# LPMP/BDD

Measured on AMD Instinct MI355X. Metric: parallel-MMA iterations/sec, 10.5M BDD nodes, 1 GPU (+ achieved HBM GB/s in roofline), higher is better.
Workload: dtype f32

## Files before the change

bdd_amd/capi.py:

```python
from __future__ import annotations

import ctypes as C
import os
import subprocess

_HERE = os.path.dirname(os.path.abspath(__file__))
LIB_PATH = os.path.abspath(os.environ["BDDMMA_LIB"]) if os.environ.get("BDDMMA_LIB") else os.path.join(_HERE, "csrc", "libbdd_mma_hip.so")

OK = 0
ERR_INVALID_ARGUMENT, ERR_INVALID_BDD, ERR_DEVICE, ERR_STATE, ERR_UNSUPPORTED, ERR_IO = -1, -2, -3, -4, -5, -6
F32, F64 = 0, 1
K_FORWARD_MM, K_BACKWARD_MM, K_FINISH_DELTA, K_OTHER, K_COUNT = 0, 1, 2, 3, 4


class Options(C.Structure):
    _fields_ = [("pack_width", C.c_uint32), ("wide_pack_width", C.c_uint32), ("deterministic", C.c_uint32),
                ("vars_per_bin", C.c_uint32), ("stage_cap", C.c_uint32), ("waves_per_block", C.c_uint32),
                ("keep_bdd_order", C.c_uint32), ("resident_sweeps", C.c_uint32), ("exchange_by_variable", C.c_uint32),
                ("variant_flags", C.c_uint32), ("pack_fill", C.c_uint32), ("pack_stagger", C.c_uint32)]


class LbfgsParams(C.Structure):
    _fields_ = [("history_size", C.c_int32), ("init_step_size", C.c_double), ("req_rel_lb_increase", C.c_double),
                ("step_size_decrease_factor", C.c_double), ("step_size_increase_factor", C.c_double)]
# ... 5 lines not shown
                ("last_kind", C.c_int32), ("last_trials", C.c_int32)]


class RunResult(C.Structure):
    _fields_ = [("iterations", C.c_uint64), ("lb_initial", C.c_double), ("lb_final", C.c_double),
                ("seconds", C.c_double), ("stop_reason", C.c_int32)]


class Profile(C.Structure):
    _fields_ = [("launches", C.c_uint64 * K_COUNT), ("total_ms", C.c_double * K_COUNT)]


_V, _U64, _I, _D = C.c_void_p, C.c_uint64, C.c_int, C.c_double
SIGNATURES = {
    "bddmma_create": (_I, [C.POINTER(_V), _I, _I, _V, _V, _U64, _V, _U64, C.POINTER(Options)]),
    "bddmma_destroy": (None, [_V]),
    "bddmma_device_count": (_I, []),
    "bddmma_device_chip": (_I, [_I, C.POINTER(C.c_uint32), C.POINTER(C.c_uint32), C.POINTER(C.c_uint64)]),
    "bddmma_set_layout_threads": (_I, [_I]),
    "bddmma_set_thread_layout_threads": (_I, [_I]),
    "bddmma_last_error": (C.c_char_p, [_V]),
    "bddmma_nr_variables": (_U64, [_V]),
    "bddmma_nr_bdds": (_U64, [_V]),
    "bddmma_nr_layers": (_U64, [_V]),
    "bddmma_nr_bdd_nodes": (_U64, [_V]),
    "bddmma_nr_hops": (_U64, [_V]),
    "bddmma_nr_packs": (_U64, [_V]),
    "bddmma_solve_sweep_kind": (_I, [_V]),
    "bddmma_fused_small": (_I, [_V]),
    "bddmma_fused_small_learned": (_I, [_V]),
    "bddmma_fused_small_history": (_I, [_V]),
    "bddmma_nontemporal_loads": (_I, [_V]),
    "bddmma_potentials_on_chip": (_I, [_V]),
    "bddmma_precision": (_I, [_V]),
    "bddmma_device": (_I, [_V]),
    "bddmma_num_bdds_per_var": (_I, [_V, _V]),
    "bddmma_layer_variables": (_I, [_V, _V]),
    "bddmma_layer_bdds": (_I, [_V, _V]),
    "bddmma_nodes_per_hop": (_I, [_V, _V]),
    "bddmma_layers_per_hop": (_I, [_V, _V]),
    "bddmma_update_costs": (_I, [_V, _V, _U64, _V, _U64, _I, _I]),
    "bddmma_set_cost": (_I, [_V, _D, _U64]),
    "bddmma_get_solver_costs": (_I, [_V, _V, _V, _V, _I]),
    "bddmma_set_solver_costs": (_I, [_V, _V, _V, _V, _I]),
    "bddmma_primal_objective_vec": (_I, [_V, _V, _I]),
    "bddmma_forward_run": (_I, [_V]),
    "bddmma_backward_run": (_I, [_V]),
    "bddmma_lower_bound": (_I, [_V, C.POINTER(_D)]),
    "bddmma_lower_bound_per_bdd": (_I, [_V, _V, _I]),
    "bddmma_iteration": (_I, [_V, _D]),
    "bddmma_iterations": (_I, [_V, _D, _U64]),
    "bddmma_learned_iterations": (_I, [_V, _V, _I, _U64, _D, _D, _V, _V, _V, _U64, _D, _I, C.POINTER(_U64)]),
    "bddmma_learned_iterations_omega_vec": (_I, [_V, _V, _I, _U64, _V, _I, _D, _V, _V, _V, _U64, _D, _I, C.POINTER(_U64)]),
    "bddmma_isotropic_dist_weights": (_I, [_V, _V, _I]),
    "bddmma_forward_mm": (_I, [_V, _D, _V, _I]),
    "bddmma_backward_mm": (_I, [_V, _D, _V, _I]),
    "bddmma_normalize_delta": (_I, [_V, _V, _I]),
    "bddmma_distribute_delta": (_I, [_V]),
    "bddmma_get_delta": (_I, [_V, _V, _I]),
    "bddmma_set_delta": (_I, [_V, _V, _I]),
    "bddmma_min_marginals": (_I, [_V, _I, _V, _V, _V, _I]),
    "bddmma_min_marginal_diff": (_I, [_V, _V, _I]),
    "bddmma_sum_marginals": (_I, [_V, _I, _I, _V, _V, _V, _I]),
    "bddmma_smooth_solution": (_I, [_V, _V, _I]),
    "bddmma_grad_min_marginal_diff": (_I, [_V, _V, _V, _V, _I]),
    "bddmma_grad_lower_bound_per_bdd": (_I, [_V, _V, _V, _V, _I, _I]),
# ... 119 lines not shown
```

bdd_amd/csrc/capi.cpp:

```cpp
#include <chrono>
#include <cmath>
#include <cstdio>
#include <cstdlib>
#include <cstring>
#include <limits>
#include <new>
#include <string>
#include <vector>

#include "../../include/bdd_mma.h"
#include "layout.hpp"
#include "solver.hpp"

using namespace bddmma;

struct bddmma_lbfgs;
extern "C" int bddmma_lbfgs_iteration(bddmma_lbfgs* l);
extern "C" int bddmma_lbfgs_update_costs(bddmma_lbfgs* l, const void* lo, uint64_t n_lo, const void* hi, uint64_t n_hi, int elem_precision,
                                         int on_device);

namespace {
thread_local std::string g_err;

template <typename F>
// ... 101 lines not shown
{
    if (n < 0) return BDDMMA_ERR_INVALID_ARGUMENT;
    set_layout_threads((unsigned)n);
    return BDDMMA_OK;
}
int bddmma_set_thread_layout_threads(int n)
{
    if (n < 0) return BDDMMA_ERR_INVALID_ARGUMENT;
    set_thread_layout_threads((unsigned)n);
    return BDDMMA_OK;
}

void bddmma_destroy(bddmma_solver* s)
{
    if (!s) return;
    delete s->impl;
    delete s;
}

const char* bddmma_last_error(const bddmma_solver* s) { return (s && s->impl) ? s->impl->err.c_str() : g_err.c_str(); }

uint64_t bddmma_nr_variables(const bddmma_solver* s) { return s && s->impl ? s->impl->n_vars : 0; }
uint64_t bddmma_nr_bdds(const bddmma_solver* s) { return s && s->impl ? s->impl->n_bdds : 0; }
uint64_t bddmma_nr_layers(const bddmma_solver* s) { return s && s->impl ? s->impl->n_layers : 0; }
uint64_t bddmma_nr_bdd_nodes(const bddmma_solver* s) { return s && s->impl ? s->impl->n_input_nodes : 0; }
uint64_t bddmma_nr_hops(const bddmma_solver* s) { return s && s->impl ? s->impl->n_hops : 0; }
uint64_t bddmma_nr_packs(const bddmma_solver* s) { return s && s->impl ? s->impl->n_packs_narrow + s->impl->n_packs_wide : 0; }
int bddmma_solve_sweep_kind(const bddmma_solver* s) { return s && s->impl ? s->impl->solve_sweep_kind : -1; }
int bddmma_fused_small(const bddmma_solver* s) { return s && s->impl ? (s->impl->fused_small ? 1 : 0) : -1; }
int bddmma_fused_small_learned(const bddmma_solver* s) { return s && s->impl ? (s->impl->fused_small_learned ? 1 : 0) : -1; }
int bddmma_fused_small_history(const bddmma_solver* s) { return s && s->impl ? (s->impl->fused_small_history ? 1 : 0) : -1; }
int bddmma_nontemporal_loads(const bddmma_solver* s) { return s && s->impl ? (s->impl->nt_loads ? 1 : 0) : -1; }
int bddmma_potentials_on_chip(const bddmma_solver* s) { return s && s->impl ? (s->impl->pot_on_chip ? 1 : 0) : -1; }
int bddmma_precision(const bddmma_solver* s) { return s && s->impl ? s->impl->precision : -1; }
int bddmma_device(const bddmma_solver* s) { return s && s->impl ? s->impl->device : -1; }
uint64_t bddmma_device_bytes(const bddmma_solver* s) { return s && s->impl ? s->impl->dev_bytes : 0; }
uint64_t bddmma_device_allocated_bytes(const bddmma_solver* s) { return s && s->impl ? s->impl->dev_alloc_bytes : 0; }

int bddmma_num_bdds_per_var(const bddmma_solver* s, int32_t* out)
{
    return guarded(s, [&](SolverBase* b) { return copy_host(b->h_nbdds, out); });
}
int bddmma_layer_variables(const bddmma_solver* s, int32_t* out)
{
    return guarded(s, [&](SolverBase* b) { return copy_host(b->h_layer_var, out); });
}
int bddmma_layer_bdds(const bddmma_solver* s, int32_t* out)
{
    return guarded(s, [&](SolverBase* b) { return copy_host(b->h_layer_bdd, out); });
}
int bddmma_nodes_per_hop(const bddmma_solver* s, uint64_t* out)
{
    return guarded(s, [&](SolverBase* b) { return copy_host(b->nodes_per_hop, out); });
}
int bddmma_layers_per_hop(const bddmma_solver* s, uint64_t* out)
{
    return guarded(s, [&](SolverBase* b) { return copy_host(b->layers_per_hop, out); });
}

int bddmma_update_costs(bddmma_solver* s, const void* lo, uint64_t n_lo, const void* hi, uint64_t n_hi,
                        int elem_precision, int on_device)
{
    return guarded(s, [&](SolverBase* b) {
        if (elem_precision != BDDMMA_F32 && elem_precision != BDDMMA_F64) {
            b->err = "elem_precision must be BDDMMA_F32 or BDDMMA_F64";
            return BDDMMA_ERR_INVALID_ARGUMENT;
// ... 670 lines not shown
```

bdd_amd/csrc/kernels/narrow4.hpp:

```cpp
#pragma once

namespace bddmma {

template <typename REAL, int WPB, int HC, bool REBUILD_T, bool STORE_F>
__device__ __forceinline__ void fwd_narrow4_body(const DevPtrs<REAL>& d, const PackDev& pk, const uint32_t* __restrict__ lrec,
                                                 const uint32_t* __restrict__ lrec_off, uint32_t lrec_words, REAL omega, uint32_t block_id)
{
    static_assert(HC + 1 <= (int)HOP_WIN, "one window of hop offsets has to hold the pack");
    constexpr int W = N3_W;
    constexpr uint32_t S = sizeof(REAL);
    constexpr uint32_t BUF = (W + 128) * S;
    using P2 = typename Pair<REAL>::type;
    extern __shared__ __attribute__((aligned(16))) unsigned char dyn_lds[];
    P2* sD = reinterpret_cast<P2*>(dyn_lds);
    __shared__ __attribute__((aligned(16))) unsigned char sF_[WPB][2][BUF];
    __shared__ __attribute__((aligned(16))) unsigned char sT_[WPB][2][BUF];
    __shared__ uint32_t sOffN_[WPB][HOP_WIN], sOffL_[WPB][HOP_WIN], sOffR_[WPB][HOP_WIN];
    const uint32_t tid = threadIdx.x;
    const int wave = __builtin_amdgcn_readfirstlane((int)(tid >> 6));
    const int lane = tid & 63;
    unsigned char* sFw = &sF_[wave][0][0];
    unsigned char* sTw = &sT_[wave][0][0];
    const uint32_t n_quads = (pk.n_packs + WPB - 1) / WPB;
    const uint32_t quad = block_to_pack(block_id, n_quads, pk.xcd_chunk);
    BDDMMA_EXIT_IF(quad >= n_quads, d)
    const uint32_t p = quad * WPB + wave;
    const bool has_pack = p < pk.n_packs;
    const uint32_t* const hp = pk.hdr_pack + 8 * (size_t)(has_pack ? p : 0);
    const uint32_t q0 = !has_pack ? 0 : hp[4];
    const uint32_t hops = !has_pack ? 0 : (hp[5] & 0xFFFFu);
    const uint32_t q1 = q0 + hops;
    const uint32_t rbase = has_pack ? lrec_off[p] : 0;
    const uint32_t c0_h = pk.hdr_quad[4 * (size_t)quad], cnt = pk.hdr_quad[4 * (size_t)quad + 1];
    BDDMMA_STAMP(p, 0);
    const REAL INF = inf_v<REAL>();
    const uint32_t slot_first = !has_pack ? 0 : hp[0], l0 = !has_pack ? 0 : hp[2];
    NarrowRs<REAL> rs(d);
    rs.rebase_layers(d, l0);
    uint32_t ent[STAGE_ITERS], esl[STAGE_ITERS];
    stage_load_tables<REAL, WPB, BDDMMA_LD_TAB_AUX>(ent, esl, rs, c0_h, cnt, tid);
    REAL* const Tp = d.T + slot_first;
    REAL* const Fp = d.F + slot_first;
    const REAL* const lohi_p = d.lohi + 2 * (size_t)l0;
    const rsrc_t rr = make_rsrc(lrec, lrec_words);
    HopWindow hw{sOffN_[wave], sOffL_[wave], sOffR_[wave], q0, q1, slot_first, l0};
    uint32_t o[HC + 4];
    uint32_t lb[HC + 1];
    P2 L[HC];
    P2 T[HC + 2];
#pragma unroll
    for (int i = 0; i < HC + 4; ++i) o[i] = 0;
#pragma unroll
    for (int i = 0; i < HC + 1; ++i) lb[i] = 0;
#pragma unroll
    for (int i = 0; i < HC + 2; ++i) T[i] = P2{REAL(0), REAL(0)};
    auto ldrec = [&](uint32_t h) { return __builtin_amdgcn_raw_buffer_load_b128(rr, (uint32_t)lane * 16u, (rbase + h * 64u) * 16u, 0); };
    const uint32_t sink = (W + 2 * (uint32_t)lane) * S;
    u4v rA = u4v{0u, 0u, 0u, 0u}, rB = rA;
    const uint32_t db = (uint32_t)wave * pk.stage_cap * (uint32_t)sizeof(P2);
    if (has_pack) {
        hw.fill(pk, q0, lane);
#pragma unroll
        for (int i = 0; i < HC + 4; ++i) o[i] = hw.node_off(q0 + i);
#pragma unroll
        for (int i = 0; i < HC + 1; ++i) lb[i] = hw.layer_off(q0 + i);
#pragma unroll
        for (int h = 0; h < HC; ++h)
            hop_load(L[h], rs.lohi, (uint32_t)h < hops ? (uint32_t)lane * (uint32_t)sizeof(P2) : OOB, lb[h] * (uint32_t)sizeof(P2));
        if constexpr (!REBUILD_T) {
#pragma unroll
            for (int h = 1; h < HC; ++h) pot_pair_load<REAL, false>(T[h], hop_rsrc(Tp, o[h], o[h + 1] - o[h]), 2u * (uint32_t)lane * S, o[h] * S);
        }
#pragma unroll
        for (int r = 0; r < 2; ++r) {
            const uint32_t j = lane + 64 * r;
            lds_st<REAL>(sFw, j * S, (j < o[1] - o[0]) ? REAL(0) : INF);
        }
#pragma unroll
        for (int b = 0; b < 2; ++b) {
            lds_st<REAL>(sTw, b * BUF + sink, REAL(0));
            lds_st<REAL>(sTw, b * BUF + sink + S, INF);
        }
        wave_sync();
        if constexpr (REBUILD_T) {
            rA = ldrec(hops - 1);
            rB = ldrec(hops >= 2 ? hops - 2 : 0);
#pragma unroll
            for (int h = HC - 1; h >= 1; --h) {
                if ((uint32_t)h < hops) {
                    const u4v ra = rA;
                    rA = rB;
                    rB = ldrec(h >= 2 ? h - 2 : 0);
                    const uint32_t tc = ((h + 1) & 1) * BUF, tn = (h & 1) * BUF;
                    const P2 c = L[h];
                    const uint32_t flags = ra[2] >> 16;
                    const REAL tla = lds_ld<REAL>(sTw, tc + (ra[0] & 0xFFFFu)), tha = lds_ld<REAL>(sTw, tc + (ra[0] >> 16));
                    const REAL tlb = lds_ld<REAL>(sTw, tc + (ra[1] & 0xFFFFu)), thb = lds_ld<REAL>(sTw, tc + (ra[1] >> 16));
                    const REAL ta = rmin(c.y + tha, c.x + tla);
                    const REAL tb = rmin(c.y + thb, c.x + tlb);
                    if (flags & LREC_REAL) lds_st<REAL>(sTw, tn + (ra[2] & 0xFFFFu), ta);
                    if (flags & LREC_TWO) lds_st<REAL>(sTw, tn + (ra[2] & 0xFFFFu) + S, tb);
                    wave_sync();
                    T[h] = lds_ld<P2>(sTw, tn + 2u * (uint32_t)lane * S);
                }
            }
        } else {
            if (2u * (uint32_t)lane < o[2] - o[1]) lds_st<P2>(sTw, BUF + 2u * (uint32_t)lane * S, T[1]);
        }
        rA = ldrec(0);
        rB = ldrec(1);
    }
    stage_load_pairs<REAL, WPB>(sD, ent, esl, rs, cnt, tid);
    if (WPB > 1) __syncthreads(); else wave_sync();
    BDDMMA_STAMP(p, 1);
#pragma unroll
    for (int h = 0; h < HC; ++h) {
        if ((uint32_t)h < hops) {
            const u4v ra = rA;
            rA = rB;
            rB = ldrec(h + 2);
            const uint32_t fc = (h & 1) * BUF, fn = ((h + 1) & 1) * BUF;
            const uint32_t stg = db + (lb[h] + (uint32_t)lane) * (uint32_t)sizeof(P2);
            const P2 c = L[h];
            const uint32_t flags = ra[2] >> 16;
            REAL fa, fb;
            lds_ld2(fa, fb, sFw, fc + (ra[2] & 0xFFFFu));
            const REAL tla = lds_ld<REAL>(sTw, fn + (ra[0] & 0xFFFFu)), tha = lds_ld<REAL>(sTw, fn + (ra[0] >> 16));
            const REAL tlb = lds_ld<REAL>(sTw, fn + (ra[1] & 0xFFFFu)), thb = lds_ld<REAL>(sTw, fn + (ra[1] >> 16));
            const P2 dd = lds_ld<P2>(dyn_lds, stg);
            if (!(REBUILD_T && h == 0))
                if (2u * (uint32_t)lane < o[h + 3] - o[h + 2]) lds_st<P2>(sTw, fc + 2u * (uint32_t)lane * S, T[h + 2]);
            lds_st<P2>(sFw, fn + 2u * (uint32_t)lane * S, P2{INF, INF});
            wave_sync();
            fa = (flags & LREC_REAL) ? fa : INF;
            fb = (flags & LREC_TWO) ? fb : INF;
            const REAL m0 = rmin((fa + c.x) + tla, (fb + c.x) + tlb);
            const REAL m1 = rmin((fa + c.y) + tha, (fb + c.y) + thb);
            const REAL mm = mm_diff1(m0, m1, omega);
            P2 nc;
            nc.x = (c.x + min0(mm)) + dd.x;
            nc.y = (c.y + min0_neg(mm)) + dd.y;
            const rsrc_t rl = hop_rsrc(reinterpret_cast<const P2*>(lohi_p), lb[h], lb[h + 1] - lb[h]);
            hop_store(nc, rl, (uint32_t)lane * (uint32_t)sizeof(P2), lb[h] * (uint32_t)sizeof(P2));
            if (flags & LREC_REAL) lds_st<REAL>(dyn_lds, stg, mm);
            lds_min(reinterpret_cast<REAL*>(sFw + fn + (ra[0] & 0xFFFFu)), fa + nc.x);
            lds_min(reinterpret_cast<REAL*>(sFw + fn + (ra[0] >> 16)), fa + nc.y);
            lds_min(reinterpret_cast<REAL*>(sFw + fn + (ra[1] & 0xFFFFu)), fb + nc.x);
            lds_min(reinterpret_cast<REAL*>(sFw + fn + (ra[1] >> 16)), fb + nc.y);
            if constexpr (STORE_F) {
                const rsrc_t rf = hop_rsrc(Fp, o[h], o[h + 1] - o[h]);
                pot_store_layer<REAL>(fa, fb, (flags & LREC_TWO) != 0, rf, ra[3] & 0xFFFFu, o[h] * S, pk.nt_potentials);
            }
            wave_sync();
        }
    }
    BDDMMA_STAMP(p, 3);
    if (WPB > 1) __syncthreads(); else wave_sync();
    BDDMMA_STAMP(p, 2);
    stage_flush<REAL, WPB>(sD, ent, esl, rs, cnt, tid);
    BDDMMA_STAMP(p, 4);
}

template <typename REAL, int WPB, int HC, bool REBUILD_T, bool STORE_F>
// ... 185 lines not shown
```

bdd_amd/csrc/solver.hpp:

```cpp
#pragma once
#include <hip/hip_runtime.h>

#include <cstdint>
#include <limits>
#include <memory>
#include <string>
#include <utility>
#include <vector>

#include "../../include/bdd_mma.h"
#include "layout.hpp"

namespace bddmma {

struct SolverBase {
    int precision = BDDMMA_F32, device = -1;
    hipStream_t stream = nullptr;
    std::string err;
    uint64_t n_vars = 0, n_bdds = 0, n_layers = 0, n_hops = 0, n_input_nodes = 0, n_slots = 0;
    int solve_sweep_kind = 0;
    uint32_t pack_width = 0, wide_pack_width = 0, wide_slot_base = 0;
    uint64_t dev_bytes = 0;
    uint64_t dev_alloc_bytes = 0;
    bool fwd_valid = false, bwd_valid = false;
// ... 15 lines not shown
    bool prof_active = false;
    std::vector<std::pair<hipEvent_t, hipEvent_t>> ev_pool;
    std::vector<int> ev_class;
    size_t ev_used = 0;
    hipEvent_t ev_t0 = nullptr, ev_t1 = nullptr;
    hipEvent_t ev_order = nullptr;

    virtual ~SolverBase() {}
    virtual int forward_run() = 0;
    virtual int backward_run() = 0;
    virtual int lower_bound(double* lb) = 0;
    virtual int lower_bound_enqueue(int slot) = 0;
    virtual int lower_bound_fetch(int slot, double* lb) = 0;
    virtual int lower_bound_per_bdd(void* out, int on_device) = 0;
    virtual int iteration(double omega) = 0;
    virtual int iterations(double omega, uint64_t n)
    {
        for (uint64_t i = 0; i < n; ++i)
            if (int rc = iteration(omega)) return rc;
        return BDDMMA_OK;
    }
    virtual int learned_iterations(const void* dist_weights, int weights_on_device, uint64_t num_itr, double omega, double improvement_slope,
                                   void* sol_avg, void* lb_first_diff_avg, void* lb_second_diff_avg, uint64_t compute_history_for_itr,
                                   double history_avg_beta, int outputs_on_device, uint64_t* itr_done, const void* omega_vec,
                                   int omega_vec_on_device) = 0;
    virtual int isotropic_dist_weights(void* out, int on_device) = 0;
    double initial_lb_change = std::numeric_limits<double>::infinity();
    std::shared_ptr<int> lbfgs_attached = std::make_shared<int>(0);
    bool fused_small = false;
    bool fused_small_learned = false;
    bool fused_small_history = false;
    bool nt_loads = false;
    bool pot_on_chip = false;
    virtual int run_plain(uint64_t max_iter, double tolerance, double slope, double time_limit, int verbose, bddmma_run_result* res) = 0;
    virtual int forward_mm(double omega, void* delta, int on_device) = 0;
    virtual int backward_mm(double omega, void* delta, int on_device) = 0;
    virtual int normalize_delta(void* delta, int on_device) = 0;
    virtual int distribute_delta() = 0;
    virtual int get_delta(void* out, int on_device) = 0;
    virtual int set_delta(const void* in, int on_device) = 0;
    virtual int update_costs(const void* lo, uint64_t n_lo, const void* hi, uint64_t n_hi, int elem_precision, int on_device) = 0;
    virtual int set_cost(double c, uint64_t var) = 0;
    virtual int get_solver_costs(void* lo, void* hi, void* mm, int on_device) = 0;
    virtual int set_solver_costs(const void* lo, const void* hi, const void* mm, int on_device) = 0;
    virtual int primal_objective_vec(void* out, int on_device) = 0;
    virtual int min_marginals(int sorted, int32_t* var, void* mm0, void* mm1, int on_device) = 0;
    virtual int min_marginal_diff(void* out, int on_device) = 0;
    virtual int sum_marginals(int sorted, int log_probs, int32_t* var, void* sm0, void* sm1, int on_device) = 0;
    virtual int smooth_solution(void* out, int on_device) = 0;
    virtual int grad_min_marginal_diff(const void* grad_mm, void* grad_lo, void* grad_hi, int on_device) = 0;
    virtual int grad_lower_bound_per_bdd(const void* grad_lb, void* grad_lo, void* grad_hi, int smooth, int on_device) = 0;
    virtual int grad_distribute_delta(const void* grad_lo, const void* grad_hi, void* grad_deferred_mm, int on_device) = 0;
    virtual int grad_cost_perturbation(const void* grad_lo, const void* grad_hi, void* grad_lo_pert, void* grad_hi_pert, int on_device) = 0;
    virtual int grad_learned_iterations(const void* dist_weights, int weights_on_device, double omega, const void* omega_vec, int omega_vec_on_device,
                                        void* grad_lo, void* grad_hi, void* grad_mm, void* grad_dist_weights_out, void* grad_omega_out, uint64_t after,
                                        uint64_t n, uint64_t num_caches, int on_device) = 0;
    virtual int bdds_solution(int sorted, char* sol, int on_device) = 0;
    virtual int net_solver_costs(void* out, int on_device) = 0;
    virtual int make_dual_feasible(void* g, int on_device) = 0;
    virtual int gradient_step(const void* g, double step, int on_device) = 0;
    virtual int projection_means(const void* g_dev) = 0;
    virtual int gradient_step_projected(const void* g_dev, double step) = 0;
    virtual bool projection_fuses_lincomb() const = 0;
    virtual int projection_means_lincomb(const LinComb& lc, const void* tag) = 0;
    virtual void* stream_handle() = 0;
    struct LbfgsViews {
// ... 54 lines not shown
```

bdd_amd/csrc/solver_impl.hpp:

```cpp
#pragma once
#include <hip/hip_runtime.h>
#include <atomic>
#include <chrono>
#include <cmath>
#include <cstdio>
#include <cstdlib>
#include <cstring>
#include <limits>
#include <memory>
#include <string>
#include <thread>
#include <type_traits>
#include <vector>
#include "../../include/bdd_mma.h"
#include "kernels.hpp"
#include "layout.hpp"
#include "solver.hpp"

namespace bddmma {

static inline void cpu_relax()
{
#if defined(__x86_64__) || defined(__i386__)
    __asm__ __volatile__("pause");
// ... 442 lines not shown
                srec_words = (uint32_t)SR.rec.size();
                use_narrow2 = true;
                narrow_gen = narrow_seg;
                for (uint16_t r : L.narrow.hop_root) narrow_gen = narrow_gen || r != NO_ROOT;
            }
        }
        if (nb_.n_packs && !use_res && !wb_.n_packs && !hb_.n_packs && !narrow_seg && pack_width == 128 && (L.ex.waves_per_block == 4 || L.ex.waves_per_block == 8) &&
            !(opts && (opts->variant_flags & 0x41000u))) {
            LayerRecords LR;
            build_layer_records(L, sizeof(REAL), LR);
            const uint32_t n3_static = L.ex.waves_per_block * (4 * (128 + 128) * (uint32_t)sizeof(REAL) + 3 * 64 * 4);
            const bool forced = opts && (opts->variant_flags & 0x2000u);
            const bool shared = forced || (LR.rec.size() * sizeof(uint32_t) <= (uint64_t)L.narrow_slots * sizeof(REAL) / 2 && n_slots <= 16'000'000ull);
            if (LR.ok && shared && stage_lds + n3_static <= lds_cu - 1024) {
                if ((rc = upload(&d_lrec, LR.rec))) return rc;
                if ((rc = upload(&d_lrec_off, LR.rec_off))) return rc;
                lrec_words = (uint32_t)LR.rec.size();
                use_narrow3 = true;
                n3_nt = sizeof(REAL) == 8 && nt_potentials != 0;
            }
        }
        if (nb_.n_packs && !use_res && !use_narrow3 && !wb_.n_packs && !hb_.n_packs && !narrow_seg && !narrow_gen && pack_width == 128 &&
            (L.ex.waves_per_block == 4 || L.ex.waves_per_block == 8) && (beyond_cache || (opts && (opts->variant_flags & 0x100000u))))
#ifndef BDDMMA_EXP_NO_N12_NT
            n12_nt = !use_narrow2 || sizeof(REAL) == 8;
#else
            n12_nt = false;
#endif
        nt_loads = n3_nt || n12_nt;
        if constexpr (sizeof(REAL) == 4) {
            if (use_narrow3 && res_hdr_ok && !n3_nt && !(opts && (opts->variant_flags & 0x200000u))) {
                uint32_t max_hops = 0;
                for (uint32_t p = 0; p < nb_.n_packs; ++p) max_hops = std::max(max_hops, L.res.pack_hdr[8 * (size_t)p + 5] & 0xFFFFu);
                onchip_hc = max_hops <= 10 ? 10 : max_hops <= 16 ? 16 : 0;
                const uint32_t part = opts ? (opts->variant_flags >> 22) & 3u : 0u;
                if (onchip_hc == 16) onchip_mode = 3;
                if (part == 1 || part == 2) {
                    if (onchip_hc == 10 && wpb == 4) onchip_mode = part;
                    else onchip_hc = 0;
                }
                pot_on_chip = onchip_hc != 0;
            }
        }
        if (wb_.n_packs) {
            wide_threads = std::min<uint32_t>(1024, std::max<uint32_t>(64, ((wide_pack_width + 1) / 2 + 63) / 64 * 64));
            wide_npt = (wide_pack_width + wide_threads - 1) / wide_threads;
            wide_npt = wide_npt <= 1 ? 1 : (wide_npt <= 2 ? 2 : 4);
            wide_lds = (uint32_t)wide2_lds_bytes(sizeof(REAL), wide_pack_width, true);
            if (wide_lds > lds_cu || wide_pack_width > 4096) {
                err = "wide_pack_width " + std::to_string(wide_pack_width) + " needs " + std::to_string(wide_lds) + " B of LDS (> 160 KiB)";
                return BDDMMA_ERR_UNSUPPORTED;
            }
        }
        if (wb_.n_packs && nb_.n_packs && !use_res && !(opts && (opts->variant_flags & 1u))) {
            const uint32_t threads = 64 * wpb;
            const uint32_t npt = (wide_pack_width + threads - 1) / threads;
            const uint32_t narrow_dyn = stage_lds + seg_bytes(wpb);
            if (npt <= 4 && wide_lds <= narrow_dyn + 16 * 1024 && std::max(narrow_dyn, wide_lds) + narrow_static <= 64 * 1024) {
                mixed = true;
                mixed_npt = npt <= 1 ? 1 : (npt <= 2 ? 2 : 4);
                mixed_lds = std::max(narrow_dyn, wide_lds);
            }
        }
        if (use_res2 && res_hdr_ok && nb_.n_packs <= SMALL_MAX_PACKS && !wb_.n_packs && !hb_.n_packs && !deterministic && !entry_by_var && !big &&
            L.var_ptr.size() == n_vars + 1 && L.ex.vpos.size() == n_layers && !(opts && (opts->variant_flags & 0x80000u))) {
            const uint32_t np = nb_.n_packs;
            std::vector<uint32_t> lds_off(n_layers);
            uint32_t max_hops = 0;
            bool ok = true;
            for (uint32_t k = 0; k < (uint32_t)n_layers && ok; ++k) {
                const uint32_t l = L.var_layers[k];
                uint32_t p = 0;
                while (p < np && !(l >= L.res.pack_hdr[8 * (size_t)p + 2] && l < L.res.pack_hdr[8 * (size_t)p + 2] + L.res.pack_hdr[8 * (size_t)p + 3])) ++p;
                if (p == np || l - L.res.pack_hdr[8 * (size_t)p + 2] >= res2_nl) { ok = false; break; }
// ... 152 lines not shown
                    if (use_res && use_res2) s.res2 = bwd ? &k_bwd_res2<REAL, W, OV> : &k_fwd_res2<REAL, W, OV>;
                    else if (use_res) s.res = bwd ? &k_bwd_res<REAL, R, W, OV> : &k_fwd_res<REAL, R, W, OV>;
                    else if (use_narrow3 && w48) {
                        s.rec = bwd ? &k_bwd_narrow3<REAL, W48, false, OV> : &k_fwd_narrow3<REAL, W48, false, OV>;
                        if constexpr (sizeof(REAL) == 8)
                            if (n3_nt) s.rec = bwd ? &k_bwd_narrow3<REAL, W48, true, OV> : &k_fwd_narrow3<REAL, W48, true, OV>;
                        s.rec_tab = d_lrec; s.rec_off = d_lrec_off; s.rec_words = lrec_words;
                    } else if (use_narrow2) {
                        if (n12_nt && R == 2 && w48) s.rec = bwd ? &k_bwd_narrow2<REAL, 2, W48, false, sizeof(REAL) == 8, OV> : &k_fwd_narrow2<REAL, 2, W48, false, sizeof(REAL) == 8, OV>;
                        else if (narrow_gen) s.rec = bwd ? &k_bwd_narrow2<REAL, R, W, true, false, OV> : &k_fwd_narrow2<REAL, R, W, true, false, OV>;
                        else s.rec = bwd ? &k_bwd_narrow2<REAL, R, W, false, false, OV> : &k_fwd_narrow2<REAL, R, W, false, false, OV>;
                        s.rec_tab = d_srec; s.rec_off = d_srec_off; s.rec_words = srec_words;
                    } else if (n12_nt && R == 2 && w48) s.narrow = bwd ? &k_bwd_narrow<REAL, 2, MODE, W48, false, true, OV> : &k_fwd_narrow<REAL, 2, MODE, W48, false, true, OV>;
                    else if (!narrow_seg) s.narrow = bwd ? &k_bwd_narrow<REAL, R, MODE, W, false, false, OV> : &k_fwd_narrow<REAL, R, MODE, W, false, false, OV>;
                    else s.narrow = bwd ? &k_bwd_narrow<REAL, R, MODE, W, true, false, OV> : &k_fwd_narrow<REAL, R, MODE, W, true, false, OV>;
                });
            });
            if (mixed)
                s.mixed = {pick<64, 128, 256>(pack_width, [&](auto PW) {
                               return pick<1, 2, 4, 8>(wpb, [&](auto W) {
                                   return pick<1, 2, 4>(mixed_npt, [&](auto N) -> MixedFn {
                                       constexpr int R = PW.value / 64;
                                       return bwd ? &k_bwd_mixed<REAL, R, W.value, N.value, OV> : &k_fwd_mixed<REAL, R, W.value, N.value, OV>;
                                   });
                               });
                           }),
                           mixed_lds};
        }
        return s;
    }
    RecFn onchip_fn(bool bwd, bool rebuild, bool store) const
    {
        if (onchip_hc == 16) return pick<4, 8>(wpb, [&](auto W) -> RecFn { return &k_bwd_narrow4<REAL, W.value, 16, true, true>; });
        if (rebuild && !store)
            return pick<4, 8>(wpb, [&](auto W) -> RecFn {
                return bwd ? &k_bwd_narrow4<REAL, W.value, 10, true, false> : &k_fwd_narrow4<REAL, W.value, 10, true, false>;
            });
        if (rebuild) return bwd ? &k_bwd_narrow4<REAL, 4, 10, true, true> : &k_fwd_narrow4<REAL, 4, 10, true, true>;
        return bwd ? &k_bwd_narrow4<REAL, 4, 10, false, false> : &k_fwd_narrow4<REAL, 4, 10, false, false>;
    }
    void resolve_kernels()
    {
        for (int bwd = 0; bwd < 2; ++bwd) {
            kern.sweep[bwd][FWD_PLAIN] = resolve_sweep<FWD_PLAIN, false>(bwd);
            kern.sweep[bwd][FWD_SOLVE] = resolve_sweep<FWD_SOLVE, false>(bwd);
            kern.sweep[bwd][FWD_SOLUTION] = resolve_sweep<FWD_SOLUTION, false>(bwd);
        }
        if (onchip_hc) {
            for (int bwd = 0; bwd < 2; ++bwd) {
                Sweep s = kern.sweep[bwd][FWD_SOLVE];
                if (onchip_mode == 3 && !bwd) { kern.onchip[0] = s; continue; }
                const bool rebuild = onchip_mode == 0 || (onchip_mode == 1) == !bwd;
                const bool store = onchip_mode != 0 && rebuild;
                if constexpr (sizeof(REAL) == 4) s.rec = onchip_fn(bwd, rebuild, onchip_mode == 3 || store);
                s.reads_pot = !rebuild;
                s.stores_pot = onchip_mode == 3 || store;
                kern.onchip[bwd] = s;
            }
        }
        kern.ex_threads = exch_small ? EXS_THREADS : exch_medium ? EXM_THREADS : EX_THREADS;
        pick<EXS_THREADS, EXM_THREADS, EX_THREADS>(kern.ex_threads, [&](auto T_) {
            constexpr int T = T_.value, U = T == EXS_THREADS ? EXS_UNROLL : T == EXM_THREADS ? EXM_UNROLL : EX_UNROLL,
                          N = T == EXS_THREADS ? EXS_NPT : T == EXM_THREADS ? EXM_NPT : EX_NPT;
            kern.ex[0] = {&k_exchange_reduce<REAL, BDDMMA_EX_ACC, EX_ITER, T, U, N, false>, exch_lds};
            kern.ex[1] = {&k_exchange_reduce<REAL, BDDMMA_EX_ACC, EX_ITER, T, U, N, true>, exch_lds};
            kern.ex_w = {&k_exchange_reduce<REAL, BDDMMA_EX_ACC, EX_ITER, T, U, N, false, true>, exch_lds};
// ... 1161 lines not shown
    {
        const uint64_t n4 = BDDMMA_TRIAD_BYTES / 16;
        stream_v4 *a = nullptr, *b = nullptr, *c = nullptr;
        HIPCHK(hipMalloc(&a, BDDMMA_TRIAD_BYTES));
        HIPCHK(hipMalloc(&b, BDDMMA_TRIAD_BYTES));
        HIPCHK(hipMalloc(&c, BDDMMA_TRIAD_BYTES));
        HIPCHK(hipMemsetAsync(b, 0, BDDMMA_TRIAD_BYTES, stream));
        HIPCHK(hipMemsetAsync(c, 0, BDDMMA_TRIAD_BYTES, stream));
        const unsigned grid = (unsigned)((n4 + 255) / 256);
        auto once = [&]() {
            if (copy) k_stream<true><<<grid, 256, 0, stream>>>(a, b, c, 3.0f, n4);
            else k_stream<false><<<grid, 256, 0, stream>>>(a, b, c, 3.0f, n4);
        };
        once();
        HIPCHK(hipEventRecord(ev_t0, stream));
        for (uint64_t i = 0; i < reps; ++i) once();
        HIPCHK(hipEventRecord(ev_t1, stream));
        HIPCHK(hipEventSynchronize(ev_t1));
        float f = 0.f;
        HIPCHK(hipEventElapsedTime(&f, ev_t0, ev_t1));
        *ms = f;
        HIPCHK(hipFree(a));
        HIPCHK(hipFree(b));
        HIPCHK(hipFree(c));
        return BDDMMA_OK;
    }

    int time_kernel(int kind, uint64_t reps, double* ms) override
    {
        HIPCHK(hipSetDevice(device));
        if (kind >= 13 && kind <= 17) return gi_time_kernel(kind, reps, ms);
        int rc = BDDMMA_OK;
        auto once = [&]() -> int {
            switch (kind) {
                case 0: return launch_fwd(FWD_PLAIN, nullptr, REAL(0), BDDMMA_K_OTHER);
                case 1: return launch_bwd(BWD_PLAIN, nullptr, REAL(0), BDDMMA_K_OTHER);
                case 2: return launch_fwd(FWD_SOLVE, d_delta_lay, REAL(0.5), BDDMMA_K_OTHER);
                case 3: return launch_bwd(BWD_SOLVE, d_delta_lay, REAL(0.5), BDDMMA_K_OTHER);
                case 4: return exchange();
                case 5: launch_bcast(d_delta_c, d_delta_lay_c); return BDDMMA_OK;
                case 8: return sm_launch_fwd();
                case 9: return sm_launch_bwd();
                case 10: return gr_launch_down();
                case 11: return gr_launch_up();
                case 12: { const int r = gr_launch_down(); return r ? r : gr_launch_up(); }
                default: err = "unknown kernel kind"; return BDDMMA_ERR_INVALID_ARGUMENT;
            }
        };
        if (kind == 6 || kind == 7) return time_stream(kind == 7, reps, ms);
        if ((kind == 8 || kind == 9) && (rc = sm_prepare())) return rc;
        if (kind == 9 && (rc = sm_launch_fwd())) return rc;
        if (kind >= 10 && kind <= 12) {
            if ((rc = gr_prepare()) || (rc = forward_run()) || (rc = backward_run())) return rc;
            HIPCHK(hipMemsetAsync(d_gr_in0, 0, n_layers * sizeof(REAL), stream));
            if (kind == 11 && (rc = gr_launch_down())) return rc;
        }
        if ((rc = once())) return rc;
        HIPCHK(hipEventRecord(ev_t0, stream));
        for (uint64_t i = 0; i < reps; ++i)
            if ((rc = once())) return rc;
        HIPCHK(hipEventRecord(ev_t1, stream));
        HIPCHK(hipEventSynchronize(ev_t1));
        float f = 0.f;
        HIPCHK(hipEventElapsedTime(&f, ev_t0, ev_t1));
        *ms = f;
        costs_changed();
        x_layer_valid = false;
#ifdef BDDMMA_STAMPS
        if (const char* path = std::getenv("BDDMMA_STAMPS_FILE")) {
            const size_t slots = 0x100000u + 65536u * 16u;
            unsigned long long* d_st = nullptr;
            HIPCHK(hipMalloc((void**)&d_st, slots * 8 * sizeof(unsigned long long)));
            HIPCHK(hipMemset(d_st, 0, slots * 8 * sizeof(unsigned long long)));
            HIPCHK(hipMemcpyToSymbol(HIP_SYMBOL(g_bddmma_stamps), &d_st, sizeof(d_st)));
            HIPCHK(hipStreamSynchronize(stream));
            rc = once();
            HIPCHK(hipStreamSynchronize(stream));
            unsigned long long* null_ = nullptr;
            HIPCHK(hipMemcpyToSymbol(HIP_SYMBOL(g_bddmma_stamps), &null_, sizeof(null_)));
            std::vector<unsigned long long> h(slots * 8);
            HIPCHK(hipMemcpy(h.data(), d_st, h.size() * sizeof(unsigned long long), hipMemcpyDeviceToHost));
            (void)hipFree(d_st);
            if (FILE* f2 = std::fopen((std::string(path) + "." + std::to_string(kind)).c_str(), "w")) {
                for (size_t sl = 0; sl < slots; ++sl)
                    if (h[sl * 8] != 0)
                        std::fprintf(f2, "%zu %llu %llu %llu %llu %llu\n", sl, h[sl * 8], h[sl * 8 + 1], h[sl * 8 + 2], h[sl * 8 + 3], h[sl * 8 + 4]);
                std::fclose(f2);
            }
            if (rc) return rc;
        }
#endif
        return BDDMMA_OK;
    }
};

}
```

bdd_amd/solver.py:

```python
from __future__ import annotations

import ctypes as C

import numpy as np

from . import capi
from .bdd_collection import BddCollection


def _ptr(a):
    return a.ctypes.data_as(C.c_void_p) if a is not None else None


def _is_dev(x):
    return hasattr(x, "data_ptr") and bool(getattr(x, "is_cuda", False))


def _dev_ptr(x, n, dtype):
    assert x.is_contiguous() and x.numel() >= n, "device buffer too small or not contiguous"
    assert x.element_size() == np.dtype(dtype).itemsize, "device buffer has the wrong element type"
    return C.c_void_p(x.data_ptr())


class bdd_hip_parallel_mma:
# ... 30 lines not shown
            self._h = None

    def __del__(self):
        try:
            self.close()
        except Exception:
            pass

    def _ck(self, rc):
        capi.check(rc, self._h)

    def nr_variables(self): return int(self._L.bddmma_nr_variables(self._h))
    def nr_layers(self): return int(self._L.bddmma_nr_layers(self._h))
    def nr_bdd_nodes(self): return int(self._L.bddmma_nr_bdd_nodes(self._h))
    def nr_hops(self): return int(self._L.bddmma_nr_hops(self._h))
    def nr_packs(self): return int(self._L.bddmma_nr_packs(self._h))

    SWEEP_KINDS = ("none", "mixed", "streaming1", "streaming2", "streaming3", "resident1", "resident2")

    def solve_sweep_kind(self) -> str:
        return self.SWEEP_KINDS[int(self._L.bddmma_solve_sweep_kind(self._h))]
    def fused_small(self) -> bool:
        return bool(self._L.bddmma_fused_small(self._h))
    def fused_small_learned(self) -> bool:
        return bool(self._L.bddmma_fused_small_learned(self._h))
    def fused_small_history(self) -> bool:
        return bool(self._L.bddmma_fused_small_history(self._h))

    def nontemporal_loads(self) -> bool:
        return bool(self._L.bddmma_nontemporal_loads(self._h))

    def potentials_on_chip(self) -> bool:
        return bool(self._L.bddmma_potentials_on_chip(self._h))
    def device(self) -> int:
        return int(self._L.bddmma_device(self._h))
    def device_bytes(self): return int(self._L.bddmma_device_bytes(self._h))
    def device_allocated_bytes(self): return int(self._L.bddmma_device_allocated_bytes(self._h))

    def nr_bdds(self, var=None):
        if var is None:
            return int(self._L.bddmma_nr_bdds(self._h))
        return int(self.get_num_bdds_per_var()[var])

    def get_num_bdds_per_var(self):
        out = np.zeros(self.nr_variables(), np.int32)
        self._ck(self._L.bddmma_num_bdds_per_var(self._h, _ptr(out)))
        return out

    def get_primal_variable_index(self):
        out = np.zeros(self.nr_layers(), np.int32)
        self._ck(self._L.bddmma_layer_variables(self._h, _ptr(out)))
        return out

    def get_bdd_index(self):
        out = np.zeros(self.nr_layers(), np.int32)
        self._ck(self._L.bddmma_layer_bdds(self._h, _ptr(out)))
        return out

    def nodes_per_hop(self):
        out = np.zeros(self.nr_hops(), np.uint64)
        self._ck(self._L.bddmma_nodes_per_hop(self._h, _ptr(out)))
        return out

    def layers_per_hop(self):
        out = np.zeros(self.nr_hops(), np.uint64)
        self._ck(self._L.bddmma_layers_per_hop(self._h, _ptr(out)))
# ... 562 lines not shown
```

include/bdd_mma.h:

```cpp
#ifndef BDD_MMA_H
#define BDD_MMA_H

#include <stddef.h>
#include <stdint.h>

#ifdef __cplusplus
extern "C" {
#endif

#define BDDMMA_OK 0
#define BDDMMA_ERR_INVALID_ARGUMENT (-1)
#define BDDMMA_ERR_INVALID_BDD (-2)
#define BDDMMA_ERR_DEVICE (-3)
#define BDDMMA_ERR_STATE (-4)
#define BDDMMA_ERR_UNSUPPORTED (-5)
#define BDDMMA_ERR_IO (-6)

#define BDDMMA_F32 0
#define BDDMMA_F64 1

typedef struct bddmma_instruction {
    uint64_t lo;
    uint64_t hi;
    uint64_t index;
// ... 22 lines not shown

int bddmma_create(bddmma_solver** out, int precision, int device,
                  const bddmma_instruction* instr, const uint64_t* bdd_delims, uint64_t n_bdds,
                  const double* costs_hi, uint64_t n_costs, const bddmma_options* opts);
void bddmma_destroy(bddmma_solver* s);

int bddmma_device_count(void);
int bddmma_device_chip(int device, uint32_t* n_cus, uint32_t* lds_bytes_per_cu, uint64_t* max_resident_threads);
int bddmma_set_layout_threads(int n);
int bddmma_set_thread_layout_threads(int n);
const char* bddmma_last_error(const bddmma_solver* s);

uint64_t bddmma_nr_variables(const bddmma_solver* s);
uint64_t bddmma_nr_bdds(const bddmma_solver* s);
uint64_t bddmma_nr_layers(const bddmma_solver* s);
uint64_t bddmma_nr_bdd_nodes(const bddmma_solver* s);
uint64_t bddmma_nr_hops(const bddmma_solver* s);
uint64_t bddmma_nr_packs(const bddmma_solver* s);
enum {
    BDDMMA_SWEEPS_NONE = 0,
    BDDMMA_SWEEPS_MIXED = 1,
    BDDMMA_SWEEPS_STREAMING1 = 2,
    BDDMMA_SWEEPS_STREAMING2 = 3,
    BDDMMA_SWEEPS_STREAMING3 = 4,
    BDDMMA_SWEEPS_RESIDENT1 = 5,
    BDDMMA_SWEEPS_RESIDENT2 = 6
};
int bddmma_solve_sweep_kind(const bddmma_solver* s);
int bddmma_fused_small(const bddmma_solver* s);
int bddmma_fused_small_learned(const bddmma_solver* s);
int bddmma_fused_small_history(const bddmma_solver* s);
int bddmma_nontemporal_loads(const bddmma_solver* s);
int bddmma_potentials_on_chip(const bddmma_solver* s);
int bddmma_precision(const bddmma_solver* s);
int bddmma_device(const bddmma_solver* s);
int bddmma_num_bdds_per_var(const bddmma_solver* s, int32_t* out);
int bddmma_layer_variables(const bddmma_solver* s, int32_t* out);
int bddmma_layer_bdds(const bddmma_solver* s, int32_t* out);
int bddmma_nodes_per_hop(const bddmma_solver* s, uint64_t* out);
int bddmma_layers_per_hop(const bddmma_solver* s, uint64_t* out);

int bddmma_update_costs(bddmma_solver* s, const void* lo, uint64_t n_lo, const void* hi, uint64_t n_hi,
                        int elem_precision, int on_device);
int bddmma_set_cost(bddmma_solver* s, double c, uint64_t var);
int bddmma_get_solver_costs(const bddmma_solver* s, void* lo, void* hi, void* deferred_mm_diff, int on_device);
int bddmma_set_solver_costs(bddmma_solver* s, const void* lo, const void* hi, const void* deferred_mm_diff, int on_device);
int bddmma_primal_objective_vec(bddmma_solver* s, void* out, int on_device);

int bddmma_forward_run(bddmma_solver* s);
int bddmma_backward_run(bddmma_solver* s);
int bddmma_lower_bound(bddmma_solver* s, double* lb);
int bddmma_lower_bound_per_bdd(bddmma_solver* s, void* out, int on_device);

int bddmma_iteration(bddmma_solver* s, double omega);
int bddmma_iterations(bddmma_solver* s, double omega, uint64_t n);
int bddmma_forward_mm(bddmma_solver* s, double omega, void* delta_lo_hi, int on_device);
int bddmma_backward_mm(bddmma_solver* s, double omega, void* delta_lo_hi, int on_device);
int bddmma_normalize_delta(const bddmma_solver* s, void* delta_lo_hi, int on_device);
int bddmma_distribute_delta(bddmma_solver* s);
int bddmma_get_delta(const bddmma_solver* s, void* out, int on_device);
int bddmma_set_delta(bddmma_solver* s, const void* in, int on_device);

int bddmma_learned_iterations(bddmma_solver* s, const void* dist_weights, int weights_on_device, uint64_t num_itr, double omega,
                              double improvement_slope, void* sol_avg, void* lb_first_diff_avg, void* lb_second_diff_avg,
                              uint64_t compute_history_for_itr, double history_avg_beta, int outputs_on_device, uint64_t* itr_done);
int bddmma_learned_iterations_omega_vec(bddmma_solver* s, const void* dist_weights, int weights_on_device, uint64_t num_itr, const void* omega_vec,
// ... 135 lines not shown
```

Baseline: 9570.

## Cache gathered T potentials in registers and add 12-hop on-chip variant

In the rebuild-T path of the narrow4 forward kernel, the backward rebuild loop now keeps the four gathered T values per hop in a register array. The forward pass reuses them instead of re-reading LDS and re-storing T rows. A 12-hop on-chip specialization is added between the existing 10 and 16 variants, so packs with 11-12 hops can use the cheaper non-storing kernel. This trades extra VGPRs (4*HC values) for fewer LDS loads and stores, which may lower occupancy. Stamp instrumentation and an accessor for the chosen hop count are also added.

```diff
diff --git a/bdd_amd/capi.py b/bdd_amd/capi.py
--- a/bdd_amd/capi.py
+++ b/bdd_amd/capi.py
@@ -61,6 +61,7 @@
     "bddmma_fused_small_history": (_I, [_V]),
     "bddmma_nontemporal_loads": (_I, [_V]),
     "bddmma_potentials_on_chip": (_I, [_V]),
+    "bddmma_onchip_hops": (_I, [_V]),
     "bddmma_precision": (_I, [_V]),
     "bddmma_device": (_I, [_V]),
     "bddmma_num_bdds_per_var": (_I, [_V, _V]),
diff --git a/bdd_amd/csrc/capi.cpp b/bdd_amd/csrc/capi.cpp
--- a/bdd_amd/csrc/capi.cpp
+++ b/bdd_amd/csrc/capi.cpp
@@ -157,6 +157,7 @@
 int bddmma_fused_small_history(const bddmma_solver* s) { return s && s->impl ? (s->impl->fused_small_history ? 1 : 0) : -1; }
 int bddmma_nontemporal_loads(const bddmma_solver* s) { return s && s->impl ? (s->impl->nt_loads ? 1 : 0) : -1; }
 int bddmma_potentials_on_chip(const bddmma_solver* s) { return s && s->impl ? (s->impl->pot_on_chip ? 1 : 0) : -1; }
+int bddmma_onchip_hops(const bddmma_solver* s) { return s && s->impl ? s->impl->onchip_hops : -1; }
 int bddmma_precision(const bddmma_solver* s) { return s && s->impl ? s->impl->precision : -1; }
 int bddmma_device(const bddmma_solver* s) { return s && s->impl ? s->impl->device : -1; }
 uint64_t bddmma_device_bytes(const bddmma_solver* s) { return s && s->impl ? s->impl->dev_bytes : 0; }
diff --git a/bdd_amd/csrc/kernels/narrow4.hpp b/bdd_amd/csrc/kernels/narrow4.hpp
--- a/bdd_amd/csrc/kernels/narrow4.hpp
+++ b/bdd_amd/csrc/kernels/narrow4.hpp
@@ -48,12 +48,18 @@
     uint32_t lb[HC + 1];
     P2 L[HC];
     P2 T[HC + 2];
+    REAL G[HC][4];
 #pragma unroll
     for (int i = 0; i < HC + 4; ++i) o[i] = 0;
 #pragma unroll
     for (int i = 0; i < HC + 1; ++i) lb[i] = 0;
-#pragma unroll
-    for (int i = 0; i < HC + 2; ++i) T[i] = P2{REAL(0), REAL(0)};
+    if constexpr (REBUILD_T) {
+#pragma unroll
+        for (int i = 0; i < HC; ++i) G[i][0] = G[i][1] = G[i][2] = G[i][3] = REAL(0);
+    } else {
+#pragma unroll
+        for (int i = 0; i < HC + 2; ++i) T[i] = P2{REAL(0), REAL(0)};
+    }
     auto ldrec = [&](uint32_t h) { return __builtin_amdgcn_raw_buffer_load_b128(rr, (uint32_t)lane * 16u, (rbase + h * 64u) * 16u, 0); };
     const uint32_t sink = (W + 2 * (uint32_t)lane) * S;
     u4v rA = u4v{0u, 0u, 0u, 0u}, rB = rA;
@@ -86,24 +92,27 @@
             rA = ldrec(hops - 1);
             rB = ldrec(hops >= 2 ? hops - 2 : 0);
 #pragma unroll
-            for (int h = HC - 1; h >= 1; --h) {
+            for (int h = HC - 1; h >= 0; --h) {
                 if ((uint32_t)h < hops) {
                     const u4v ra = rA;
                     rA = rB;
                     rB = ldrec(h >= 2 ? h - 2 : 0);
                     const uint32_t tc = ((h + 1) & 1) * BUF, tn = (h & 1) * BUF;
-                    const P2 c = L[h];
-                    const uint32_t flags = ra[2] >> 16;
                     const REAL tla = lds_ld<REAL>(sTw, tc + (ra[0] & 0xFFFFu)), tha = lds_ld<REAL>(sTw, tc + (ra[0] >> 16));
                     const REAL tlb = lds_ld<REAL>(sTw, tc + (ra[1] & 0xFFFFu)), thb = lds_ld<REAL>(sTw, tc + (ra[1] >> 16));
-                    const REAL ta = rmin(c.y + tha, c.x + tla);
-                    const REAL tb = rmin(c.y + thb, c.x + tlb);
-                    if (flags & LREC_REAL) lds_st<REAL>(sTw, tn + (ra[2] & 0xFFFFu), ta);
-                    if (flags & LREC_TWO) lds_st<REAL>(sTw, tn + (ra[2] & 0xFFFFu) + S, tb);
-                    wave_sync();
-                    T[h] = lds_ld<P2>(sTw, tn + 2u * (uint32_t)lane * S);
+                    G[h][0] = tla, G[h][1] = tha, G[h][2] = tlb, G[h][3] = thb;
+                    if (h >= 1) {
+                        const P2 c = L[h];
+                        const uint32_t flags = ra[2] >> 16;
+                        const REAL ta = rmin(c.y + tha, c.x + tla);
+                        const REAL tb = rmin(c.y + thb, c.x + tlb);
+                        if (flags & LREC_REAL) lds_st<REAL>(sTw, tn + (ra[2] & 0xFFFFu), ta);
+                        if (flags & LREC_TWO) lds_st<REAL>(sTw, tn + (ra[2] & 0xFFFFu) + S, tb);
+                        wave_sync();
+                    }
                 }
             }
+            BDDMMA_STAMP(p, 5);
         } else {
             if (2u * (uint32_t)lane < o[2] - o[1]) lds_st<P2>(sTw, BUF + 2u * (uint32_t)lane * S, T[1]);
         }
@@ -125,10 +134,15 @@
             const uint32_t flags = ra[2] >> 16;
             REAL fa, fb;
             lds_ld2(fa, fb, sFw, fc + (ra[2] & 0xFFFFu));
-            const REAL tla = lds_ld<REAL>(sTw, fn + (ra[0] & 0xFFFFu)), tha = lds_ld<REAL>(sTw, fn + (ra[0] >> 16));
-            const REAL tlb = lds_ld<REAL>(sTw, fn + (ra[1] & 0xFFFFu)), thb = lds_ld<REAL>(sTw, fn + (ra[1] >> 16));
+            REAL tla, tha, tlb, thb;
+            if constexpr (REBUILD_T) {
+                tla = G[h][0], tha = G[h][1], tlb = G[h][2], thb = G[h][3];
+            } else {
+                tla = lds_ld<REAL>(sTw, fn + (ra[0] & 0xFFFFu)), tha = lds_ld<REAL>(sTw, fn + (ra[0] >> 16));
+                tlb = lds_ld<REAL>(sTw, fn + (ra[1] & 0xFFFFu)), thb = lds_ld<REAL>(sTw, fn + (ra[1] >> 16));
+            }
             const P2 dd = lds_ld<P2>(dyn_lds, stg);
-            if (!(REBUILD_T && h == 0))
+            if constexpr (!REBUILD_T)
                 if (2u * (uint32_t)lane < o[h + 3] - o[h + 2]) lds_st<P2>(sTw, fc + 2u * (uint32_t)lane * S, T[h + 2]);
             lds_st<P2>(sFw, fn + 2u * (uint32_t)lane * S, P2{INF, INF});
             wave_sync();
diff --git a/bdd_amd/csrc/solver.hpp b/bdd_amd/csrc/solver.hpp
--- a/bdd_amd/csrc/solver.hpp
+++ b/bdd_amd/csrc/solver.hpp
@@ -71,6 +71,7 @@
     bool fused_small_history = false;
     bool nt_loads = false;
     bool pot_on_chip = false;
+    int onchip_hops = 0;
     virtual int run_plain(uint64_t max_iter, double tolerance, double slope, double time_limit, int verbose, bddmma_run_result* res) = 0;
     virtual int forward_mm(double omega, void* delta, int on_device) = 0;
     virtual int backward_mm(double omega, void* delta, int on_device) = 0;
diff --git a/bdd_amd/csrc/solver_impl.hpp b/bdd_amd/csrc/solver_impl.hpp
--- a/bdd_amd/csrc/solver_impl.hpp
+++ b/bdd_amd/csrc/solver_impl.hpp
@@ -498,7 +498,7 @@
             if (use_narrow3 && res_hdr_ok && !n3_nt && !(opts && (opts->variant_flags & 0x200000u))) {
                 uint32_t max_hops = 0;
                 for (uint32_t p = 0; p < nb_.n_packs; ++p) max_hops = std::max(max_hops, L.res.pack_hdr[8 * (size_t)p + 5] & 0xFFFFu);
-                onchip_hc = max_hops <= 10 ? 10 : max_hops <= 16 ? 16 : 0;
+                onchip_hc = max_hops <= 10 ? 10 : max_hops <= 12 ? 12 : max_hops <= 16 ? 16 : 0;
                 const uint32_t part = opts ? (opts->variant_flags >> 22) & 3u : 0u;
                 if (onchip_hc == 16) onchip_mode = 3;
                 if (part == 1 || part == 2) {
@@ -506,6 +506,7 @@
                     else onchip_hc = 0;
                 }
                 pot_on_chip = onchip_hc != 0;
+                onchip_hops = onchip_hc;
             }
         }
         if (wb_.n_packs) {
@@ -724,6 +725,10 @@
     RecFn onchip_fn(bool bwd, bool rebuild, bool store) const
     {
         if (onchip_hc == 16) return pick<4, 8>(wpb, [&](auto W) -> RecFn { return &k_bwd_narrow4<REAL, W.value, 16, true, true>; });
+        if (onchip_hc == 12)
+            return pick<4, 8>(wpb, [&](auto W) -> RecFn {
+                return bwd ? &k_bwd_narrow4<REAL, W.value, 12, true, false> : &k_fwd_narrow4<REAL, W.value, 12, true, false>;
+            });
         if (rebuild && !store)
             return pick<4, 8>(wpb, [&](auto W) -> RecFn {
                 return bwd ? &k_bwd_narrow4<REAL, W.value, 10, true, false> : &k_fwd_narrow4<REAL, W.value, 10, true, false>;
@@ -1951,6 +1956,10 @@
         if (kind >= 13 && kind <= 17) return gi_time_kernel(kind, reps, ms);
         int rc = BDDMMA_OK;
         auto once = [&]() -> int {
+#ifdef BDDMMA_STAMPS
+            if ((kind == 2 || kind == 3) && onchip_hc && std::getenv("BDDMMA_STAMPS_ONCHIP"))
+                return launch_sweep(kind == 3, kern.onchip[kind - 2], d_delta_lay, REAL(0.5), BDDMMA_K_OTHER);
+#endif
             switch (kind) {
                 case 0: return launch_fwd(FWD_PLAIN, nullptr, REAL(0), BDDMMA_K_OTHER);
                 case 1: return launch_bwd(BWD_PLAIN, nullptr, REAL(0), BDDMMA_K_OTHER);
@@ -2003,7 +2012,7 @@
             if (FILE* f2 = std::fopen((std::string(path) + "." + std::to_string(kind)).c_str(), "w")) {
                 for (size_t sl = 0; sl < slots; ++sl)
                     if (h[sl * 8] != 0)
-                        std::fprintf(f2, "%zu %llu %llu %llu %llu %llu\n", sl, h[sl * 8], h[sl * 8 + 1], h[sl * 8 + 2], h[sl * 8 + 3], h[sl * 8 + 4]);
+                        std::fprintf(f2, "%zu %llu %llu %llu %llu %llu %llu\n", sl, h[sl * 8], h[sl * 8 + 1], h[sl * 8 + 2], h[sl * 8 + 3], h[sl * 8 + 4], h[sl * 8 + 5]);
                 std::fclose(f2);
             }
             if (rc) return rc;
diff --git a/bdd_amd/solver.py b/bdd_amd/solver.py
--- a/bdd_amd/solver.py
+++ b/bdd_amd/solver.py
@@ -86,6 +86,9 @@
 
     def potentials_on_chip(self) -> bool:
         return bool(self._L.bddmma_potentials_on_chip(self._h))
+
+    def onchip_hops(self) -> int:
+        return int(self._L.bddmma_onchip_hops(self._h))
     def device(self) -> int:
         return int(self._L.bddmma_device(self._h))
     def device_bytes(self): return int(self._L.bddmma_device_bytes(self._h))
diff --git a/include/bdd_mma.h b/include/bdd_mma.h
--- a/include/bdd_mma.h
+++ b/include/bdd_mma.h
@@ -78,6 +78,7 @@
 int bddmma_fused_small_history(const bddmma_solver* s);
 int bddmma_nontemporal_loads(const bddmma_solver* s);
 int bddmma_potentials_on_chip(const bddmma_solver* s);
+int bddmma_onchip_hops(const bddmma_solver* s);
 int bddmma_precision(const bddmma_solver* s);
 int bddmma_device(const bddmma_solver* s);
 int bddmma_num_bdds_per_var(const bddmma_solver* s, int32_t* out);
```

Result: faster. 9745 (median of 6 runs) (+1.8%).
